# reazon-research/ReazonSpeech

Measured on AMD Instinct MI355X. Metric: RTFx (audio-sec/wall-sec), FastConformer-RNNT 619M batch=256, higher is better.
Workload: dtype bf16

## Files before the change

### reazonspeech_amd/csrc/k_rnnt.hip

```cpp
#include <cstdio>
#include <cstdlib>

#include "k_rnnt_common.h"

namespace {

__global__ void rnnt_init_kernel(DecodeState st, const int32_t* __restrict__ enc_lens, int B, int blank,
                                 int32_t* __restrict__ n_ids) {
    __shared__ int n_alive_s;
    if (threadIdx.x == 0) n_alive_s = 0;
    __syncthreads();
    for (int b = threadIdx.x; b < B; b += blockDim.x) {
        st.tcur[b] = 0; st.sym[b] = 0; st.token[b] = blank; st.act[b] = b;
        if (st.token2) st.token2[b] = -1;
        n_ids[b] = 0;
        if (enc_lens[b] > 0) st.alive[atomicAdd(&n_alive_s, 1)] = b;
    }
    __syncthreads();
    if (threadIdx.x == 0) { st.counters[0] = B; st.counters[1] = 0; st.counters[2] = n_alive_s; st.counters[3] = 0; }
}

__global__ __launch_bounds__(1024) void rnnt_lstm_kernel(DecodeState st, int layer, int B, int H,
                                                        const float* __restrict__ embed,
                                                        const float* __restrict__ W ,
// ... 335 lines not shown
        for (int ctile = lane; ctile < n_ctiles; ctile += 64) {
            const float ov = st.pmax[row * n_ctiles + ctile];
            const int oi = st.pidx[row * n_ctiles + ctile];
            if (ov > val || (ov == val && oi < idx)) { val = ov; idx = oi; }
        }
#pragma unroll
        for (int off = 32; off > 0; off >>= 1) {
            const float ov = __shfl_xor(val, off, 64);
            const int oi = __shfl_xor(idx, off, 64);
            if (ov > val || (ov == val && oi < idx)) { val = ov; idx = oi; }
        }
        if (idx == blank || idx == st.unk || idx == 0x7fffffff) { t += 1; sy = 0; continue; }
        if (lane == 0) {
            const int n = n_ids[b];
            if (n < u_max) { ids[(size_t)b * u_max + n] = idx; frames[(size_t)b * u_max + n] = t; n_ids[b] = n + 1; }
            else st.counters[1] = 1;
            if (st.token2) st.token2[b] = st.token[b];
            st.token[b] = idx;
        }
        emitted = true;
        sy += 1;
        if (sy >= max_symbols) { t += 1; sy = 0; }
        break;
    }
    if (lane != 0) return;
    st.tcur[b] = t; st.sym[b] = sy;
    if (t < T) {
        const int pos = atomicAdd(&st.counters[2 + ((step + 1) & 1)], 1);
        st.alive[(size_t)((step + 1) & 1) * B + pos] = b;
        if (emitted) { const int pa = atomicAdd(&st.counters[0], 1); st.act[pa] = b; }
    }
}

__global__ __launch_bounds__(1024) void rnnt_lstm4_kernel(DecodeState st, int layer, int B, int H,
                                                         const float* __restrict__ embed,
                                                         const float* __restrict__ W4 ,
                                                         const float* __restrict__ bias ) {
    __shared__ float part[SPLITK_LSTM][32][17];
    __shared__ int rows_s[32];
    const int n_act = st.counters[0];
    const int rt = blockIdx.y, ug = blockIdx.x;
    if (rt * 32 >= n_act) return;
    const int tid = threadIdx.x, lane = tid & 63, wave = tid >> 6;
    if (tid < 32) {
        const int i = rt * 32 + tid;
        rows_s[tid] = st.act[i < n_act ? i : n_act - 1];
    }
    __syncthreads();
    const int li = lane & 15, kk = lane >> 4;
    const int lr = lane >> 2, lc = lane & 3;
    const int perm = 4 * (4 * li + kk);
    const int K = 2 * H, kslice = K / SPLITK_LSTM, nkb = K / 16;
    const float* xsrc[2];
    const float* hsrc[2];
#pragma unroll
    for (int ri = 0; ri < 2; ++ri) {
        const int row = rows_s[ri * 16 + lr];
        xsrc[ri] = layer == 0 ? embed + (size_t)st.token[row] * H : st.h_tmp + ((size_t)(layer - 1) * B + row) * H;
        hsrc[ri] = st.h + ((size_t)layer * B + row) * H;
    }
    const float* wfrag = W4 + ((size_t)ug * nkb) * 256 + lane * 4;
    f32x4_t acc[2] = {(f32x4_t){0.f, 0.f, 0.f, 0.f}, (f32x4_t){0.f, 0.f, 0.f, 0.f}};
    const int kbeg = wave * kslice, nblk = kslice / 16;
    float4 av[2][8], wv[8];
#pragma unroll
    for (int u = 0; u < 8; ++u)
        if (u < nblk) {
            const int k = kbeg + 16 * u + 4 * lc;
#pragma unroll
            for (int ri = 0; ri < 2; ++ri)
                av[ri][u] = (k < H) ? *reinterpret_cast<const float4*>(xsrc[ri] + k) : *reinterpret_cast<const float4*>(hsrc[ri] + (k - H));
            wv[u] = *reinterpret_cast<const float4*>(wfrag + (size_t)((kbeg >> 4) + u) * 256);
        }
#pragma unroll
    for (int u = 0; u < 8; ++u)
        if (u < nblk) {
            const float4 a0 = to_mfma_a_layout(av[0][u], perm), a1 = to_mfma_a_layout(av[1][u], perm);
#define RS_MFMA_E(c)                                                                         \
            acc[0] = __builtin_amdgcn_mfma_f32_16x16x4f32(a0.c, wv[u].c, acc[0], 0, 0, 0);   \
            acc[1] = __builtin_amdgcn_mfma_f32_16x16x4f32(a1.c, wv[u].c, acc[1], 0, 0, 0);
            RS_MFMA_E(x) RS_MFMA_E(y) RS_MFMA_E(z) RS_MFMA_E(w)
#undef RS_MFMA_E
        }
#pragma unroll
    for (int ri = 0; ri < 2; ++ri)
#pragma unroll
        for (int r = 0; r < 4; ++r) part[wave][ri * 16 + 4 * kk + r][li] = acc[ri][r];
    __syncthreads();
    if (tid >= 128) return;
    const int i = tid >> 2, u4 = tid & 3;
    if (rt * 32 + i >= n_act) return;
    const int brow = rows_s[i];
    const int unit = ug * 4 + u4;
    float z[4];
#pragma unroll
    for (int gt = 0; gt < 4; ++gt) {
        float sm = part[0][i][gt * 4 + u4];
#pragma unroll
        for (int sl = 1; sl < SPLITK_LSTM; ++sl) sm = sm + part[sl][i][gt * 4 + u4];
        z[gt] = sm + bias[gt * H + unit];
    }
    const float ig = rs_sigmoidf(z[0]), fg = rs_sigmoidf(z[1]), gg = rs_tanhf(z[2]), og = rs_sigmoidf(z[3]);
    const size_t o = ((size_t)layer * B + brow) * H + unit;
    const float cn = fmaf(fg, st.c[o], ig * gg);
    st.c_tmp[o] = cn;
    st.h_tmp[o] = og * rs_tanhf(cn);
}

__global__ __launch_bounds__(512) void rnnt_pred16_kernel(DecodeState st, int B, int L, int H, int N ,
                                                         const float* __restrict__ W, const float* __restrict__ bias) {
    __shared__ float part[SPLITK_TILE][32][17];
    __shared__ int rows_s[32];
    const int rt = blockIdx.y, ct = blockIdx.x;
    const int tid = threadIdx.x, lane = tid & 63, wave = tid >> 6;
    const int n_rows = st.counters[0];
    if (rt * 32 >= n_rows) return;
    if (tid < 32) {
        const int i = rt * 32 + tid;
        rows_s[tid] = st.act[i < n_rows ? i : n_rows - 1];
    }
    __syncthreads();
    const int li = lane & 15, kk = lane >> 4;
    const int lr = lane >> 2, lc = lane & 3;
    const int perm = 4 * (4 * li + kk);
    const int K = H, nkb = K / 16;
    const float* asrc[2];
#pragma unroll
    for (int ri = 0; ri < 2; ++ri) asrc[ri] = st.h_tmp + ((size_t)(L - 1) * B + rows_s[ri * 16 + lr]) * H;
    const float* wfrag = W + ((size_t)ct * nkb) * 256 + lane * 4;
    f32x4_t acc[2] = {(f32x4_t){0.f, 0.f, 0.f, 0.f}, (f32x4_t){0.f, 0.f, 0.f, 0.f}};
    const int kslice = K / SPLITK_TILE, kbeg = wave * kslice, nblk = kslice / 16;
    float4 av[2][8], wv[8];
#pragma unroll
    for (int u = 0; u < 8; ++u)
        if (u < nblk) {
            const int k = kbeg + 16 * u + 4 * lc;
#pragma unroll
            for (int ri = 0; ri < 2; ++ri) av[ri][u] = *reinterpret_cast<const float4*>(asrc[ri] + k);
            wv[u] = *reinterpret_cast<const float4*>(wfrag + (size_t)((kbeg >> 4) + u) * 256);
        }
#pragma unroll
    for (int u = 0; u < 8; ++u)
        if (u < nblk) {
            const float4 a0 = to_mfma_a_layout(av[0][u], perm), a1 = to_mfma_a_layout(av[1][u], perm);
#define RS_MFMA_E(c)                                                                         \
            acc[0] = __builtin_amdgcn_mfma_f32_16x16x4f32(a0.c, wv[u].c, acc[0], 0, 0, 0);   \
            acc[1] = __builtin_amdgcn_mfma_f32_16x16x4f32(a1.c, wv[u].c, acc[1], 0, 0, 0);
            RS_MFMA_E(x) RS_MFMA_E(y) RS_MFMA_E(z) RS_MFMA_E(w)
#undef RS_MFMA_E
        }
#pragma unroll
    for (int ri = 0; ri < 2; ++ri)
#pragma unroll
        for (int r = 0; r < 4; ++r) part[wave][ri * 16 + 4 * kk + r][li] = acc[ri][r];
    __syncthreads();
    const int i = tid >> 4, c = tid & 15;
    const bool row_ok = rt * 32 + i < n_rows;
    const int brow = rows_s[i];
    const int v = ct * 16 + c;
    if (row_ok && v < N) {
        float sm = part[0][i][c];
#pragma unroll
        for (int sl = 1; sl < SPLITK_TILE; ++sl) sm = sm + part[sl][i][c];
        st.g[(size_t)brow * N + v] = sm + bias[v];
    }
    if (row_ok) {
        const int nct = gridDim.x;
        for (int l = 0; l < L; ++l)
            for (int u = ct * 16 + c; u < H; u += nct * 16) {
                const size_t o = ((size_t)l * B + brow) * H + u;
                st.h[o] = st.h_tmp[o];
                st.c[o] = st.c_tmp[o];
            }
    }
}

__global__ __launch_bounds__(256) void rnnt_prep_kernel(DecodeState st, const float* __restrict__ f, int B, int Tp, int J,
                                                        int step) {
    const int lane = threadIdx.x & 63;
    const int slot = blockIdx.x * 4 + (threadIdx.x >> 6);
    if (blockIdx.x == 0 && threadIdx.x == 0) {
        st.counters[0] = 0;
        st.counters[2 + ((step + 1) & 1)] = 0;
    }
    if (slot >= st.counters[2 + (step & 1)]) return;
    const int b = st.alive[(size_t)(step & 1) * B + slot];
    int t = st.tcur[b];
    t = t < Tp ? t : Tp - 1;
    const float* fr = f + ((size_t)b * Tp + t) * J;
    const float* gr = st.g + (size_t)b * J;
    float ss = 0.0f;
    for (int k = 4 * lane; k < J; k += 256) {
        const float4 fv = *reinterpret_cast<const float4*>(fr + k), gv = *reinterpret_cast<const float4*>(gr + k);
        float a0, a1, a2, a3;
        if (st.joint_act) {
            a0 = rs_tanhf(fv.x + gv.x); a1 = rs_tanhf(fv.y + gv.y); a2 = rs_tanhf(fv.z + gv.z); a3 = rs_tanhf(fv.w + gv.w);
        } else {
            a0 = fmaxf(fv.x + gv.x, 0.0f); a1 = fmaxf(fv.y + gv.y, 0.0f); a2 = fmaxf(fv.z + gv.z, 0.0f); a3 = fmaxf(fv.w + gv.w, 0.0f);
        }
        ss = fmaf(a0, a0, fmaf(a1, a1, fmaf(a2, a2, fmaf(a3, a3, ss))));
        *reinterpret_cast<u16x4_t*>(st.a16 + (size_t)slot * J + k) = pack_bf16x4(a0, a1, a2, a3);
    }
    ss = wave_sum(ss);
    if (lane == 0) st.anorm[slot] = sqrtf(ss) * 1.0001f;
}

__global__ __launch_bounds__(256) void rnnt_screen_kernel(DecodeState st, const float* __restrict__ f, int B, int Tp, int J,
                                                          int Vpad, const uint16_t* __restrict__ W16,
                                                          const float* __restrict__ bpad, int step) {
    extern __shared__ __attribute__((aligned(16))) char scr_smem[];
    const int ldrow = J * 2 + 16;
    const int ct = blockIdx.x, rt = blockIdx.y;
    const int tid = threadIdx.x, lane = tid & 63, wave = tid >> 6;
    const int n_alive = st.counters[2 + (step & 1)];
    if (rt * 32 >= n_alive) return;
    const int col0 = (ct * 4 + wave) * 16;
    const bool has_cols = col0 < Vpad;
    const int li = lane & 15, kc = lane >> 4;
    const int nks = J / 32;
    const uint16_t* wrow = W16 + (size_t)((has_cols ? col0 : 0) + li) * J + kc * 8;
    bf16x8_t wf[20];
#pragma unroll
    for (int q = 0; q < 20; ++q)
        if (q < nks) wf[q] = *reinterpret_cast<const bf16x8_t*>(wrow + q * 32);
    const float bv = bpad[(has_cols ? col0 : 0) + li];
    {
        const int per_row = J / 8;
        for (int idx = tid; idx < 32 * per_row; idx += 256) {
            const int r = idx / per_row, c = idx - r * per_row;
            const int i = rt * 32 + r;
            const uint4 v = *reinterpret_cast<const uint4*>(st.a16 + (size_t)(i < n_alive ? i : n_alive - 1) * J + c * 8);
            *reinterpret_cast<uint4*>(scr_smem + r * ldrow + c * 16) = v;
        }
    }
    __syncthreads();
    if (!has_cols) return;
    f32x4_t acc[2] = {(f32x4_t){0.f, 0.f, 0.f, 0.f}, (f32x4_t){0.f, 0.f, 0.f, 0.f}};
#pragma unroll
    for (int q = 0; q < 20; ++q)
        if (q < nks) {
#pragma unroll
            for (int ri = 0; ri < 2; ++ri) {
                const bf16x8_t af = *reinterpret_cast<const bf16x8_t*>(scr_smem + (ri * 16 + li) * ldrow + (q * 32 + kc * 8) * 2);
                acc[ri] = __builtin_amdgcn_mfma_f32_16x16x32_bf16(af, wf[q], acc[ri], 0, 0, 0);
            }
        }
#pragma unroll
    for (int ri = 0; ri < 2; ++ri)
#pragma unroll
        for (int r = 0; r < 4; ++r) {
            const int slot = rt * 32 + ri * 16 + 4 * kc + r;
            if (slot < n_alive) st.zapprox[(size_t)slot * Vpad + col0 + li] = acc[ri][r] + bv;
        }
}

constexpr int VER_CAP = 1024;

__device__ __forceinline__ void verify_evaluate(const int* cand_s, int n_cand, const float* a_s, const float* __restrict__ Wrm,
                                                const float* __restrict__ bo, int J, int lane, float& best, int& best_idx) {
    const int cgrp = lane >> 3, sl = lane & 7;
    const int kslice = J / SPLITK_TILE, nblk = kslice / 16;
    for (int c0 = 0; c0 < n_cand; c0 += 8) {
        const bool valid = c0 + cgrp < n_cand;
        const int cand = valid ? cand_s[c0 + cgrp] : 0;
        const float* w = Wrm + (size_t)cand * J + sl * kslice;
        const float* as = a_s + sl * kslice;
        float4 wv[8][4];
#pragma unroll
        for (int u = 0; u < 8; ++u)
            if (u < nblk) {
#pragma unroll
                for (int kk = 0; kk < 4; ++kk) wv[u][kk] = *reinterpret_cast<const float4*>(w + 16 * u + 4 * kk);
            }
        float acc = 0.0f;
#pragma unroll
        for (int u = 0; u < 8; ++u)
            if (u < nblk) {
                float4 av[4];
#pragma unroll
                for (int kk = 0; kk < 4; ++kk) av[kk] = *reinterpret_cast<const float4*>(as + 16 * u + 4 * kk);
#define RS_CHAIN_E(cc) _Pragma("unroll") for (int kk = 0; kk < 4; ++kk) acc = fmaf(av[kk].cc, wv[u][kk].cc, acc);
                RS_CHAIN_E(x) RS_CHAIN_E(y) RS_CHAIN_E(z) RS_CHAIN_E(w)
#undef RS_CHAIN_E
            }
        float sum = __shfl(acc, lane & ~7, 64);
#pragma unroll
// ... 150 lines not shown
    int n_cand = 0;
#pragma unroll
    for (int c = 0; c < NCHW; ++c) {
        const bool is = zr[c] >= thr;
        const unsigned long long mask = __ballot(is);
        if (is) cand_s[n_cand + __builtin_popcountll(mask & ((1ull << lane) - 1ull))] = (wave * NCHW + c) * 64 + lane;
        n_cand += __builtin_popcountll(mask);
    }
    __builtin_amdgcn_fence(__ATOMIC_ACQ_REL, "wavefront");
    __builtin_amdgcn_wave_barrier();
    float best = -INFINITY;
    int best_idx = 0x7fffffff;
    verify_evaluate(cand_s, n_cand, a_s, Wrm, bo, J, lane, best, best_idx);
    if (lane == 0) { red[4 + wave] = best; reinterpret_cast<int*>(red)[8 + wave] = best_idx; }
    __syncthreads();
    if (threadIdx.x != 0) return;
#pragma unroll
    for (int w = 0; w < 4; ++w) {
        const float v = red[4 + w];
        const int i = reinterpret_cast<int*>(red)[8 + w];
        if (v > best || (v == best && i < best_idx)) { best = v; best_idx = i; }
    }
    verify_commit(st, b, t, best_idx, enc_lens, B, blank, max_symbols, u_max, step, ids, frames, n_ids);
}

}


namespace {

__global__ __launch_bounds__(256) void k2_decoder_kernel(DecodeState st, int B, int D, const float* __restrict__ embed,
                                                         const float* __restrict__ conv_w ) {
    const int n_rows = st.counters[0];
    if ((int)blockIdx.x >= n_rows) return;
    const int row = st.act[blockIdx.x];
    const int t0 = st.token2[row], t1 = st.token[row];
    for (int c = threadIdx.x; c < D; c += 256) {
        const int g4 = c & ~3;
        float acc = 0.0f;
#pragma unroll
        for (int i = 0; i < 4; ++i) {
            const float e = t0 >= 0 ? embed[(size_t)t0 * D + g4 + i] : 0.0f;
            acc = fmaf(conv_w[(c * 4 + i) * 2 + 0], e, acc);
        }
#pragma unroll
        for (int i = 0; i < 4; ++i) {
            const float e = t1 >= 0 ? embed[(size_t)t1 * D + g4 + i] : 0.0f;
            acc = fmaf(conv_w[(c * 4 + i) * 2 + 1], e, acc);
        }
        st.h_tmp[(size_t)row * D + c] = fmaxf(acc, 0.0f);
    }
}

constexpr int LSTM_LDS = SPLITK_LSTM * 4 * 32 * 16 * 4 + 32 * 4;
constexpr int TILE_LDS = SPLITK_TILE * 32 * 65 * 4 + 32 * 4;

bool narrow_kernels_usable(const rs_ctx* ctx) {
    const int L = ctx->d.pred_layers, H = ctx->d.pred_hidden;
    bool narrow = ctx->decode_narrow;
    for (int l = 0; l < L; ++l) narrow = narrow && ctx->lstm_w4[l] != nullptr;
    return narrow && 2 * H / SPLITK_LSTM / 16 <= 8 && H / SPLITK_TILE / 16 <= 8;
}

void launch_lstm_pred(rs_ctx* ctx, const DecodeState& st, int B, int rows_bound, bool narrow, hipStream_t s) {
    const int L = ctx->d.pred_layers, H = ctx->d.pred_hidden, J = ctx->d.joint_hidden;
    const int rts = (rows_bound + 31) / 32 > 0 ? (rows_bound + 31) / 32 : 1;
    if (ctx->k2_conv_w) {
        hipLaunchKernelGGL(k2_decoder_kernel, dim3(rows_bound > 0 ? rows_bound : 1), dim3(256), 0, s, st, B, H, ctx->embed, ctx->k2_conv_w);
        hipLaunchKernelGGL(rnnt_pred16_kernel, dim3((J + 15) / 16, rts), dim3(512), 0, s, st, B, 1, H, J, ctx->jpred_w, ctx->jpred_b);
        return;
    }
    if (narrow) {
        for (int l = 0; l < L; ++l)
            hipLaunchKernelGGL(rnnt_lstm4_kernel, dim3(H / 4, rts), dim3(1024), 0, s, st, l, B, H, ctx->embed, ctx->lstm_w4[l],
                               ctx->lstm_b[l]);
        hipLaunchKernelGGL(rnnt_pred16_kernel, dim3((J + 15) / 16, rts), dim3(512), 0, s, st, B, L, H, J, ctx->jpred_w,
                           ctx->jpred_b);
        return;
    }
    for (int l = 0; l < L; ++l)
        hipLaunchKernelGGL(rnnt_lstm_kernel, dim3(H / 16, rts), dim3(1024), LSTM_LDS, s, st, l, B, H, ctx->embed,
                           ctx->lstm_w[l], ctx->lstm_b[l]);
    hipLaunchKernelGGL(rnnt_tile_kernel<0>, dim3((J + 63) / 64, rts), dim3(512), TILE_LDS, s, st, (const float*)nullptr, B,
                       0, L, H, H, J, ctx->jpred_w, ctx->jpred_b, 0, 0, 1);
}

int joint_grid_x(int nct, int rts) {
    return rts > 1 && !rs_knob(RS_KNOB_DECODE_NO_XCD) ? (nct + 7) / 8 * 8 : nct;
}

int ensure_decode_lds(rs_ctx* ctx) {
    if (int rc = rs_ensure_dynamic_lds(ctx, (const void*)rnnt_lstm_kernel, LSTM_LDS); rc != RS_OK) return rc;
    if (int rc = rs_ensure_dynamic_lds(ctx, (const void*)rnnt_tile_kernel<0>, TILE_LDS); rc != RS_OK) return rc;
    if (int rc = rs_ensure_dynamic_lds(ctx, (const void*)rnnt_tile_kernel<1>, TILE_LDS); rc != RS_OK) return rc;
    if (int rc = rs_ensure_dynamic_lds(ctx, (const void*)rnnt_tile_kernel<2>, TILE_LDS); rc != RS_OK) return rc;
    if (int rc = rs_ensure_dynamic_lds(ctx, (const void*)rnnt_tile_kernel<3>, TILE_LDS); rc != RS_OK) return rc;
    if (int rc = rs_ensure_dynamic_lds(ctx, (const void*)rnnt_tile_kernel<4>, TILE_LDS); rc != RS_OK) return rc;
    return rs_ensure_dynamic_lds(ctx, (const void*)rnnt_tile_kernel<5>, TILE_LDS);
}

}

int rs_rnnt_launch_lstm_pred(rs_ctx* ctx, const void* st_ptr, int rows, hipStream_t s) {
    if (int rc = ensure_decode_lds(ctx); rc != RS_OK) return rc;
    launch_lstm_pred(ctx, *reinterpret_cast<const DecodeState*>(st_ptr), rows, rows, narrow_kernels_usable(ctx), s);
    return RS_OK;
}

int rs_rnnt_launch_joint_logits(rs_ctx* ctx, const void* st_ptr, const float* joint_enc, int rows, int tp_max, int rows_per_utt,
                                int step, hipStream_t s) {
    if (int rc = ensure_decode_lds(ctx); rc != RS_OK) return rc;
    const rs_dims& d = ctx->d;
    const int nct = (d.n_logits + 63) / 64;
    hipLaunchKernelGGL(rnnt_tile_kernel<2>, dim3(joint_grid_x(nct, (rows + 31) / 32), (rows + 31) / 32), dim3(512), TILE_LDS, s,
                       *reinterpret_cast<const DecodeState*>(st_ptr), joint_enc, rows, tp_max, d.pred_layers, d.pred_hidden,
                       d.joint_hidden, d.n_logits, ctx->jout_w, ctx->jout_b, nct, step, rows_per_utt);
    return RS_OK;
}

int rs_rnnt_launch_joint_logits_indirect(rs_ctx* ctx, const void* st_ptr, const float* joint_enc, int rows, int rows_bound, int tp_max,
                                         int rows_per_utt, int step, hipStream_t s) {
    if (int rc = ensure_decode_lds(ctx); rc != RS_OK) return rc;
    const rs_dims& d = ctx->d;
    const int nct = (d.n_logits + 63) / 64;
    const int rts = (rows_bound + 31) / 32 > 0 ? (rows_bound + 31) / 32 : 1;
    const DecodeState& st = *reinterpret_cast<const DecodeState*>(st_ptr);
    if (st.a_pre)
        hipLaunchKernelGGL(rnnt_tile_kernel<4>, dim3(joint_grid_x(nct, rts), rts), dim3(512), TILE_LDS, s, st, joint_enc, rows, tp_max,
                           d.pred_layers, d.pred_hidden, d.joint_hidden, d.n_logits, ctx->jout_w, ctx->jout_b, nct, step, rows_per_utt);
    else
        hipLaunchKernelGGL(rnnt_tile_kernel<3>, dim3(joint_grid_x(nct, rts), rts), dim3(512), TILE_LDS, s, st, joint_enc, rows, tp_max,
                           d.pred_layers, d.pred_hidden, d.joint_hidden, d.n_logits, ctx->jout_w, ctx->jout_b, nct, step, rows_per_utt);
    return RS_OK;
}

constexpr int LOOKAHEAD_MAX = 8;

static void greedy_layout(const rs_ctx* ctx, int B, rs_arena& a, DecodeState& st) {
    const rs_dims& d = ctx->d;
    const size_t state = (size_t)d.pred_layers * B * d.pred_hidden, J = d.joint_hidden;
    const size_t nct = (d.n_logits + 63) / 64, Vpad = (size_t)(d.n_logits + 15) / 16 * 16;
    st.h = a.take<float>(state); st.c = a.take<float>(state);
    st.h_tmp = a.take<float>(state); st.c_tmp = a.take<float>(state);
    st.g = a.take<float>(B * J);
    st.tcur = a.take<int32_t>(B); st.sym = a.take<int32_t>(B);
    st.token = a.take<int32_t>(B); st.act = a.take<int32_t>(B);
    if (ctx->k2_conv_w) st.token2 = a.take<int32_t>(B);
    st.alive = a.take<int32_t>((size_t)2 * B);
    st.counters = a.take<int32_t>(16);
    st.pmax = a.take<float>(B * LOOKAHEAD_MAX * nct); st.pidx = a.take<int32_t>(B * LOOKAHEAD_MAX * nct);
    st.a16 = a.take<uint16_t>(B * J); st.anorm = a.take<float>(B);
    st.zapprox = a.take<float>(B * Vpad);
}
constexpr size_t GREEDY_SLACK = 1024;

size_t rs_rnnt_workspace_bytes(const rs_ctx* ctx, int B) {
    rs_arena a;
    DecodeState st{};
    greedy_layout(ctx, B, a, st);
    return a.bytes() + GREEDY_SLACK;
}

int rs_rnnt_greedy_impl(rs_ctx* ctx, const float* joint_enc, const int32_t* enc_lens, int B, int tp_max, int u_max,
                        int32_t* ids, int32_t* frames, int32_t* n_ids, void* workspace, size_t workspace_bytes,
                        hipStream_t s) {
    const rs_dims& d = ctx->d;
    const int L = d.pred_layers, H = d.pred_hidden, J = d.joint_hidden, V = d.n_logits;
    if (B <= 0) return RS_OK;
    if (H % 128 || J % 128) return rs_fail(ctx, RS_EINVAL, "rnnt: pred_hidden/joint_hidden must be multiples of 128");
    if (L < 1 || L > 4) return rs_fail(ctx, RS_EINVAL, "rnnt: 1..4 LSTM layers supported");
    rs_arena arena(workspace);
    DecodeState st{};
    greedy_layout(ctx, B, arena, st);
    if (workspace_bytes < arena.bytes() + GREEDY_SLACK) return rs_fail(ctx, RS_EWORKSPACE, "rnnt: workspace too small");
    st.joint_act = d.joint_act;
    if (ctx->k2_conv_w) st.unk = ctx->k2 ? rs_k2_unk_id(ctx) : -1;
    const size_t state_bytes = (size_t)L * B * H * 4;
    const int nct = (V + 63) / 64, Vpad = (V + 15) / 16 * 16;
    const bool screen = ctx->decode_screen && ctx->jout_w16 && ctx->jout_wrm && ctx->jout_bpad && ctx->jout_wmax &&
                        J / SPLITK_TILE / 16 <= 8 && J / 32 <= 20;

    if (int rc = ensure_decode_lds(ctx); rc != RS_OK) return rc;
    const bool narrow = narrow_kernels_usable(ctx);
    auto lstm_and_pred = [&](int rows_bound) { launch_lstm_pred(ctx, st, B, rows_bound, narrow, s); };

    rs_prof_begin(ctx, RS_PROF_DECODE, s, 0.0, 0.0);
    RS_HIP(ctx, hipMemsetAsync(st.h, 0, 2 * rs_align(state_bytes), s));
    RS_HIP(ctx, hipMemsetAsync(st.g, 0, (size_t)B * J * 4, s));
    hipLaunchKernelGGL(rnnt_init_kernel, dim3(1), dim3(256), 0, s, st, enc_lens, B, d.blank_id, n_ids);
    lstm_and_pred(B);
    RS_CHECK_LAUNCH(ctx, "rnnt init");

    const int max_steps = tp_max + (u_max < tp_max * d.max_symbols ? u_max : tp_max * d.max_symbols) + 1;
    const int CHUNK = 16;
    const bool lookahead = !rs_knob(RS_KNOB_DECODE_NO_LOOKAHEAD);
    const bool verify_wide = rs_knob(RS_KNOB_VERIFY_WIDE) != 0;
    int32_t host_counters[4] = {0, 0, 0, 0};
    int steps = 0, alive_bound = B;
    bool finished = false;
    while (!finished && steps < max_steps) {
        for (int c = 0; c < CHUNK; ++c, ++steps) {
            const int rows = alive_bound < B ? alive_bound : B;
            if (screen) {
                const int rts = (rows + 31) / 32 > 0 ? (rows + 31) / 32 : 1;
                hipLaunchKernelGGL(rnnt_prep_kernel, dim3((rows + 3) / 4 > 0 ? (rows + 3) / 4 : 1), dim3(256), 0, s, st, joint_enc, B,
                                   tp_max, J, steps);
                hipLaunchKernelGGL(rnnt_screen_kernel, dim3((Vpad + 63) / 64, rts), dim3(256), 32 * (J * 2 + 16), s, st, joint_enc, B,
                                   tp_max, J, Vpad, ctx->jout_w16, ctx->jout_bpad, steps);
                const dim3 vg((rows + 3) / 4 > 0 ? (rows + 3) / 4 : 1), vgw(rows > 0 ? rows : 1);
#define RS_VERIFY_ARGS st, joint_enc, enc_lens, B, tp_max, J, V, Vpad, ctx->jout_wrm, ctx->jout_b, ctx->jout_wmax, d.blank_id, d.max_symbols, u_max, steps, ids, frames, n_ids
                if (V > 64 * 48 && V <= 4 * 64 * 48)
                    hipLaunchKernelGGL(rnnt_verify_wide_kernel<48>, vgw, dim3(256), J * 4 + 4 * 48 * 64 * 4 + 64, s, RS_VERIFY_ARGS);
                else if (V > 64 * 48)
                    hipLaunchKernelGGL(rnnt_verify_kernel<0>, vg, dim3(256), 4 * J * 4 + 4 * VER_CAP * 4, s, RS_VERIFY_ARGS);
                else if (verify_wide)
                    hipLaunchKernelGGL(rnnt_verify_wide_kernel<12>, vgw, dim3(256), J * 4 + 4 * 12 * 64 * 4 + 64, s, RS_VERIFY_ARGS);
                else if (V <= 64 * 8)
                    hipLaunchKernelGGL(rnnt_verify_kernel<8>, vg, dim3(256), 4 * J * 4 + 4 * 8 * 64 * 4, s, RS_VERIFY_ARGS);
                else
                    hipLaunchKernelGGL(rnnt_verify_kernel<48>, vg, dim3(256), 4 * J * 4 + 4 * 48 * 64 * 4, s, RS_VERIFY_ARGS);
#undef RS_VERIFY_ARGS
            } else {
                int la = 1;
                if (lookahead) while (la < LOOKAHEAD_MAX && 2 * la * (rows > 0 ? rows : 1) <= 256) la *= 2;
                if (la > 1) {
                    const int rts = (rows * la + 31) / 32 > 0 ? (rows * la + 31) / 32 : 1;
                    hipLaunchKernelGGL(rnnt_tile_kernel<5>, dim3(joint_grid_x(nct, rts), rts), dim3(512), TILE_LDS, s, st, joint_enc, B, tp_max, L, H,
                                       J, V, ctx->jout_w, ctx->jout_b, nct, steps, la);
                    hipLaunchKernelGGL(rnnt_finalize_la_kernel, dim3((rows + 3) / 4 > 0 ? (rows + 3) / 4 : 1), dim3(256), 0, s, st, enc_lens, B, nct,
                                       d.blank_id, d.max_symbols, u_max, steps, la, ids, frames, n_ids);
                } else {
                    const int rts = (rows + 31) / 32 > 0 ? (rows + 31) / 32 : 1;
                    hipLaunchKernelGGL(rnnt_tile_kernel<1>, dim3(joint_grid_x(nct, rts), rts), dim3(512), TILE_LDS, s, st, joint_enc, B, tp_max, L, H,
                                       J, V, ctx->jout_w, ctx->jout_b, nct, steps, 1);
                    hipLaunchKernelGGL(rnnt_finalize_kernel, dim3((rows + 3) / 4 > 0 ? (rows + 3) / 4 : 1), dim3(256), 0, s, st, enc_lens, B, nct,
                                       d.blank_id, d.max_symbols, u_max, steps, ids, frames, n_ids);
                }
// ... 16 lines not shown
```

### reazonspeech_amd/csrc/rs_knobs.h

```cpp
#pragma once
#include <stdlib.h>
#include <string.h>

#include <atomic>
#include <mutex>

#include "../../include/rs_asr.h"

#define RS_KNOBS(X)                                                                                                                   \
    X(GEMM_TILE, "RS_GEMM_TILE", INT, 0, "forced GEMM tile height (256 / 192 / 128 / 64); 0 = by shape")                              \
    X(GEMM_GROUP_M, "RS_GEMM_GROUP_M", INT, 0, "row panels per XCD tile group; 0 = by shape")                                         \
    X(GEMM_PAIRS, "RS_GEMM_PAIRS", INT, 2, "2 = two tiles per workgroup, LDS ring carried over; 1 = ring restarted; 0 = one tile")    \
    X(GEMM_BREG, "RS_GEMM_BREG", INT, 0, "1 = 256- / 192-row launches keep the weight operand out of LDS (global -> VGPR)")           \
    X(ATTN_PERSIST, "RS_ATTN_PERSIST", INT, 0, "1 = full attention on resident workgroups that walk the items (n >= 2: on n)")        \
    X(ATTN_STREAM, "RS_ATTN_STREAM", INT, 0, "1 = the streaming attention form (+ 16 x mask: phases left out, for timing)")           \
    X(ATTN64, "RS_ATTN64", INT, 4, "head_dim 64: key blocks per chunk; 0 = the one-workgroup-per-CU geometry")                        \
    X(ATTN64_NW, "RS_ATTN64_NW", INT, 4, "head_dim 64: waves per workgroup (the second number of $RS_ATTN64)")                        \
    X(ATTN_F32_OLD, "RS_ATTN_F32_OLD", PRESENT, 0, "float32 attention: the first form (one wave per key sum)")                        \
    X(ATTN_F32_KEYS, "RS_ATTN_F32_KEYS", PRESENT, 0, "float32 attention: the second form (keys over lanes, no MFMA)")                 \
    X(GLU_GENERIC, "RS_GLU_GENERIC", INT, 0, "GLU + depthwise conv: 1 = the any-kernel-size path, 2 = the f32-tile kernel on the gated layout") \
    X(SUB_IM2COL, "RS_SUB_IM2COL", PRESENT, 0, "ESPnet subsampling: gather the 3 x 3 patches into a matrix first (sizes the workspace too)") \
    X(FUSE_GLU, "RS_FUSE_GLU", INT, 1, "context default: 0 = GLU in the depthwise kernel, not the pw1 GEMM epilogue")                 \
    X(DEFER_OUT_NORM, "RS_DEFER_OUT_NORM", INT, 1, "context default: 0 = every output norm stores its f32 rows")                      \
    X(DECODE_SCREEN, "RS_DECODE_SCREEN", INT, 1, "context default: 0 = exact evaluation of every joint column")                       \
    X(DECODE_NARROW, "RS_DECODE_NARROW", INT, 1, "context default: 0 = the wide-tile LSTM / projection kernels")                      \
    X(DECODE_NO_XCD, "RS_DECODE_NO_XCD", PRESENT, 0, "greedy decode: joint grids not padded to a multiple of 8 column tiles")         \
    X(DECODE_NO_LOOKAHEAD, "RS_DECODE_NO_LOOKAHEAD", PRESENT, 0, "greedy decode: one frame per utterance and step at every batch size") \
    X(VERIFY_WIDE, "RS_VERIFY_WIDE", INT, 0, "screened joint: 1 = a workgroup per row for V <= 3072 too")                             \
    X(DECODE_TRACE, "RS_DECODE_TRACE", PRESENT, 0, "greedy decode: print the step count of every call to stderr")                     \
    X(BEAM_SPEC, "RS_BEAM_SPEC", INT, 3, "beam search: evaluations asked for per iteration (1 .. 8; sizes the workspace too)")         \
    X(BEAM_TRACE, "RS_BEAM_TRACE", PRESENT, 0, "beam search: phase timing of the step kernel")                                        \
    X(BEAM_RECORD_LDS, "RS_BEAM_RECORD_LDS", PRESENT, 0, "beam search: the any-vocabulary record kernel on a small vocabulary")       \
    X(AVSR_POSCONV_OLD, "RS_AVSR_POSCONV_OLD", PRESENT, 0, "AV-HuBERT positional convolution: the VALU form")                         \
    X(K2_CONV1_OLD, "RS_K2_CONV1_OLD", PRESENT, 0, "Zipformer conv1: the VALU form (the one other channel counts run)")               \
    X(K2_ATTW_SWEEPS, "RS_K2_ATTW_SWEEPS", INT, 1, "Zipformer attention weights: 3 = the three-sweep kernel")                         \
    X(K2_CONV2_FUSED, "RS_K2_CONV2_FUSED", INT, 1, "default of option k2_conv2_fused: 0 = patch matrix + GEMM launch")                \
    X(K2_CNX_FUSED, "RS_K2_CNX_FUSED", INT, 1, "default of option k2_cnx_fused: 0 = the ConvNeXt pointwise pair as two GEMM launches")

enum rs_knob_id {
#define RS_KNOB_ENUM(id, env, kind, def, what) RS_KNOB_##id,
    RS_KNOBS(RS_KNOB_ENUM)
#undef RS_KNOB_ENUM
    RS_KNOB_COUNT
};
enum rs_knob_kind { RS_KNOB_PRESENT, RS_KNOB_INT };
struct rs_knob_row { const char* env; rs_knob_kind kind; int def; };
static const rs_knob_row rs_knob_rows[RS_KNOB_COUNT] = {
#define RS_KNOB_ROW(id, env, kind, def, what) {env, RS_KNOB_##kind, def},
    RS_KNOBS(RS_KNOB_ROW)
#undef RS_KNOB_ROW
};

struct rs_knob_table {
    std::atomic<int> value[RS_KNOB_COUNT];
    std::atomic<bool> given[RS_KNOB_COUNT];
    std::once_flag once;
};
inline rs_knob_table rs_knob_state;

inline void rs_knobs_read_env() {
// ... 38 lines not shown
```

Baseline: 46360.

## Loop decode kernels over row tiles to reuse register-held weights across tiles

```diff
diff --git a/reazonspeech_amd/csrc/k_rnnt.hip b/reazonspeech_amd/csrc/k_rnnt.hip
--- a/reazonspeech_amd/csrc/k_rnnt.hip
+++ b/reazonspeech_amd/csrc/k_rnnt.hip
@@ -391,6 +391,7 @@
     }
 }
 
+constexpr int LSTM4_NB = 5;
 __global__ __launch_bounds__(1024) void rnnt_lstm4_kernel(DecodeState st, int layer, int B, int H,
                                                          const float* __restrict__ embed,
                                                          const float* __restrict__ W4 ,
@@ -398,139 +399,163 @@
     __shared__ float part[SPLITK_LSTM][32][17];
     __shared__ int rows_s[32];
     const int n_act = st.counters[0];
-    const int rt = blockIdx.y, ug = blockIdx.x;
-    if (rt * 32 >= n_act) return;
+    const int ug = blockIdx.x;
+    if ((int)blockIdx.y * 32 >= n_act) return;
     const int tid = threadIdx.x, lane = tid & 63, wave = tid >> 6;
-    if (tid < 32) {
-        const int i = rt * 32 + tid;
-        rows_s[tid] = st.act[i < n_act ? i : n_act - 1];
-    }
-    __syncthreads();
     const int li = lane & 15, kk = lane >> 4;
     const int lr = lane >> 2, lc = lane & 3;
     const int perm = 4 * (4 * li + kk);
     const int K = 2 * H, kslice = K / SPLITK_LSTM, nkb = K / 16;
-    const float* xsrc[2];
-    const float* hsrc[2];
-#pragma unroll
-    for (int ri = 0; ri < 2; ++ri) {
-        const int row = rows_s[ri * 16 + lr];
-        xsrc[ri] = layer == 0 ? embed + (size_t)st.token[row] * H : st.h_tmp + ((size_t)(layer - 1) * B + row) * H;
-        hsrc[ri] = st.h + ((size_t)layer * B + row) * H;
-    }
-    const float* wfrag = W4 + ((size_t)ug * nkb) * 256 + lane * 4;
-    f32x4_t acc[2] = {(f32x4_t){0.f, 0.f, 0.f, 0.f}, (f32x4_t){0.f, 0.f, 0.f, 0.f}};
     const int kbeg = wave * kslice, nblk = kslice / 16;
-    float4 av[2][8], wv[8];
-#pragma unroll
-    for (int u = 0; u < 8; ++u)
-        if (u < nblk) {
-            const int k = kbeg + 16 * u + 4 * lc;
-#pragma unroll
-            for (int ri = 0; ri < 2; ++ri)
-                av[ri][u] = (k < H) ? *reinterpret_cast<const float4*>(xsrc[ri] + k) : *reinterpret_cast<const float4*>(hsrc[ri] + (k - H));
-            wv[u] = *reinterpret_cast<const float4*>(wfrag + (size_t)((kbeg >> 4) + u) * 256);
-        }
-#pragma unroll
-    for (int u = 0; u < 8; ++u)
-        if (u < nblk) {
-            const float4 a0 = to_mfma_a_layout(av[0][u], perm), a1 = to_mfma_a_layout(av[1][u], perm);
-#define RS_MFMA_E(c)                                                                         \
-            acc[0] = __builtin_amdgcn_mfma_f32_16x16x4f32(a0.c, wv[u].c, acc[0], 0, 0, 0);   \
-            acc[1] = __builtin_amdgcn_mfma_f32_16x16x4f32(a1.c, wv[u].c, acc[1], 0, 0, 0);
-            RS_MFMA_E(x) RS_MFMA_E(y) RS_MFMA_E(z) RS_MFMA_E(w)
+    int my_row = 0;
+    if (tid < 32) {
+        const int i = blockIdx.y * 32 + tid;
+        my_row = st.act[i < n_act ? i : n_act - 1];
+    }
+    constexpr int NB = LSTM4_NB;
+    const float* wfrag = W4 + ((size_t)ug * nkb + (kbeg >> 4)) * 256 + lane * 4;
+    float4 wv[NB];
+#pragma unroll
+    for (int u = 0; u < NB; ++u)
+        if (u < nblk) wv[u] = *reinterpret_cast<const float4*>(wfrag + u * 256);
+#pragma clang loop unroll(disable)
+    for (int rt = blockIdx.y; rt * 32 < n_act; rt += gridDim.y) {
+        const bool more = (rt + (int)gridDim.y) * 32 < n_act;
+        if (tid < 32) rows_s[tid] = my_row;
+        __syncthreads();
+        const float* asrc[2];
+#pragma unroll
+        for (int ri = 0; ri < 2; ++ri) {
+            const int row = rows_s[ri * 16 + lr];
+            if (kbeg < H)
+                asrc[ri] = (layer == 0 ? embed + (size_t)st.token[row] * H : st.h_tmp + ((size_t)(layer - 1) * B + row) * H) + kbeg + 4 * lc;
+            else
+                asrc[ri] = st.h + ((size_t)layer * B + row) * H + (kbeg - H) + 4 * lc;
+        }
+        f32x4_t acc[2] = {(f32x4_t){0.f, 0.f, 0.f, 0.f}, (f32x4_t){0.f, 0.f, 0.f, 0.f}};
+        float4 av[2][NB];
+#pragma unroll
+        for (int u = 0; u < NB; ++u)
+            if (u < nblk) {
+#pragma unroll
+                for (int ri = 0; ri < 2; ++ri) av[ri][u] = *reinterpret_cast<const float4*>(asrc[ri] + 16 * u);
+            }
+        if (more && tid < 32) {
+            const int i = (rt + gridDim.y) * 32 + tid;
+            my_row = st.act[i < n_act ? i : n_act - 1];
+        }
+#pragma unroll
+        for (int u = 0; u < NB; ++u)
+            if (u < nblk) {
+                const float4 a0 = to_mfma_a_layout(av[0][u], perm), a1 = to_mfma_a_layout(av[1][u], perm);
+#define RS_MFMA_E(c)                                                                             \
+                acc[0] = __builtin_amdgcn_mfma_f32_16x16x4f32(a0.c, wv[u].c, acc[0], 0, 0, 0);   \
+                acc[1] = __builtin_amdgcn_mfma_f32_16x16x4f32(a1.c, wv[u].c, acc[1], 0, 0, 0);
+                RS_MFMA_E(x) RS_MFMA_E(y) RS_MFMA_E(z) RS_MFMA_E(w)
 #undef RS_MFMA_E
-        }
-#pragma unroll
-    for (int ri = 0; ri < 2; ++ri)
-#pragma unroll
-        for (int r = 0; r < 4; ++r) part[wave][ri * 16 + 4 * kk + r][li] = acc[ri][r];
-    __syncthreads();
-    if (tid >= 128) return;
-    const int i = tid >> 2, u4 = tid & 3;
-    if (rt * 32 + i >= n_act) return;
-    const int brow = rows_s[i];
-    const int unit = ug * 4 + u4;
-    float z[4];
-#pragma unroll
-    for (int gt = 0; gt < 4; ++gt) {
-        float sm = part[0][i][gt * 4 + u4];
-#pragma unroll
-        for (int sl = 1; sl < SPLITK_LSTM; ++sl) sm = sm + part[sl][i][gt * 4 + u4];
-        z[gt] = sm + bias[gt * H + unit];
-    }
-    const float ig = rs_sigmoidf(z[0]), fg = rs_sigmoidf(z[1]), gg = rs_tanhf(z[2]), og = rs_sigmoidf(z[3]);
-    const size_t o = ((size_t)layer * B + brow) * H + unit;
-    const float cn = fmaf(fg, st.c[o], ig * gg);
-    st.c_tmp[o] = cn;
-    st.h_tmp[o] = og * rs_tanhf(cn);
+            }
+#pragma unroll
+        for (int ri = 0; ri < 2; ++ri)
+#pragma unroll
+            for (int r = 0; r < 4; ++r) part[wave][ri * 16 + 4 * kk + r][li] = acc[ri][r];
+        __syncthreads();
+        const int i = tid >> 2, u4 = tid & 3;
+        if (tid < 128 && rt * 32 + i < n_act) {
+            const int brow = rows_s[i];
+            const int unit = ug * 4 + u4;
+            float z[4];
+#pragma unroll
+            for (int gt = 0; gt < 4; ++gt) {
+                float sm = part[0][i][gt * 4 + u4];
+#pragma unroll
+                for (int sl = 1; sl < SPLITK_LSTM; ++sl) sm = sm + part[sl][i][gt * 4 + u4];
+                z[gt] = sm + bias[gt * H + unit];
+            }
+            const float ig = rs_sigmoidf(z[0]), fg = rs_sigmoidf(z[1]), gg = rs_tanhf(z[2]), og = rs_sigmoidf(z[3]);
+            const size_t o = ((size_t)layer * B + brow) * H + unit;
+            const float cn = fmaf(fg, st.c[o], ig * gg);
+            st.c_tmp[o] = cn;
+            st.h_tmp[o] = og * rs_tanhf(cn);
+        }
+        if (more) __syncthreads();
+    }
 }
 
 __global__ __launch_bounds__(512) void rnnt_pred16_kernel(DecodeState st, int B, int L, int H, int N ,
                                                          const float* __restrict__ W, const float* __restrict__ bias) {
     __shared__ float part[SPLITK_TILE][32][17];
     __shared__ int rows_s[32];
-    const int rt = blockIdx.y, ct = blockIdx.x;
+    const int ct = blockIdx.x;
     const int tid = threadIdx.x, lane = tid & 63, wave = tid >> 6;
     const int n_rows = st.counters[0];
-    if (rt * 32 >= n_rows) return;
-    if (tid < 32) {
-        const int i = rt * 32 + tid;
-        rows_s[tid] = st.act[i < n_rows ? i : n_rows - 1];
-    }
-    __syncthreads();
+    if ((int)blockIdx.y * 32 >= n_rows) return;
     const int li = lane & 15, kk = lane >> 4;
     const int lr = lane >> 2, lc = lane & 3;
     const int perm = 4 * (4 * li + kk);
     const int K = H, nkb = K / 16;
-    const float* asrc[2];
-#pragma unroll
-    for (int ri = 0; ri < 2; ++ri) asrc[ri] = st.h_tmp + ((size_t)(L - 1) * B + rows_s[ri * 16 + lr]) * H;
-    const float* wfrag = W + ((size_t)ct * nkb) * 256 + lane * 4;
-    f32x4_t acc[2] = {(f32x4_t){0.f, 0.f, 0.f, 0.f}, (f32x4_t){0.f, 0.f, 0.f, 0.f}};
     const int kslice = K / SPLITK_TILE, kbeg = wave * kslice, nblk = kslice / 16;
-    float4 av[2][8], wv[8];
+    if (tid < 32) {
+        const int i = blockIdx.y * 32 + tid;
+        rows_s[tid] = st.act[i < n_rows ? i : n_rows - 1];
+    }
+    const float* wfrag = W + ((size_t)ct * nkb + (kbeg >> 4)) * 256 + lane * 4;
+    float4 wv[8];
 #pragma unroll
     for (int u = 0; u < 8; ++u)
-        if (u < nblk) {
-            const int k = kbeg + 16 * u + 4 * lc;
-#pragma unroll
-            for (int ri = 0; ri < 2; ++ri) av[ri][u] = *reinterpret_cast<const float4*>(asrc[ri] + k);
-            wv[u] = *reinterpret_cast<const float4*>(wfrag + (size_t)((kbeg >> 4) + u) * 256);
-        }
-#pragma unroll
-    for (int u = 0; u < 8; ++u)
-        if (u < nblk) {
-            const float4 a0 = to_mfma_a_layout(av[0][u], perm), a1 = to_mfma_a_layout(av[1][u], perm);
-#define RS_MFMA_E(c)                                                                         \
-            acc[0] = __builtin_amdgcn_mfma_f32_16x16x4f32(a0.c, wv[u].c, acc[0], 0, 0, 0);   \
-            acc[1] = __builtin_amdgcn_mfma_f32_16x16x4f32(a1.c, wv[u].c, acc[1], 0, 0, 0);
-            RS_MFMA_E(x) RS_MFMA_E(y) RS_MFMA_E(z) RS_MFMA_E(w)
+        if (u < nblk) wv[u] = *reinterpret_cast<const float4*>(wfrag + u * 256);
+    for (int rt = blockIdx.y; rt * 32 < n_rows; rt += gridDim.y) {
+        const bool more = (rt + (int)gridDim.y) * 32 < n_rows;
+        if (tid < 32 && rt != (int)blockIdx.y) {
+            const int i = rt * 32 + tid;
+            rows_s[tid] = st.act[i < n_rows ? i : n_rows - 1];
+        }
+        __syncthreads();
+        const float* asrc[2];
+#pragma unroll
+        for (int ri = 0; ri < 2; ++ri) asrc[ri] = st.h_tmp + ((size_t)(L - 1) * B + rows_s[ri * 16 + lr]) * H + kbeg + 4 * lc;
+        f32x4_t acc[2] = {(f32x4_t){0.f, 0.f, 0.f, 0.f}, (f32x4_t){0.f, 0.f, 0.f, 0.f}};
+        float4 av[2][8];
+#pragma unroll
+        for (int u = 0; u < 8; ++u)
+            if (u < nblk) {
+#pragma unroll
+                for (int ri = 0; ri < 2; ++ri) av[ri][u] = *reinterpret_cast<const float4*>(asrc[ri] + 16 * u);
+            }
+#pragma unroll
+        for (int u = 0; u < 8; ++u)
+            if (u < nblk) {
+                const float4 a0 = to_mfma_a_layout(av[0][u], perm), a1 = to_mfma_a_layout(av[1][u], perm);
+#define RS_MFMA_E(c)                                                                             \
+                acc[0] = __builtin_amdgcn_mfma_f32_16x16x4f32(a0.c, wv[u].c, acc[0], 0, 0, 0);   \
+                acc[1] = __builtin_amdgcn_mfma_f32_16x16x4f32(a1.c, wv[u].c, acc[1], 0, 0, 0);
+                RS_MFMA_E(x) RS_MFMA_E(y) RS_MFMA_E(z) RS_MFMA_E(w)
 #undef RS_MFMA_E
-        }
-#pragma unroll
-    for (int ri = 0; ri < 2; ++ri)
-#pragma unroll
-        for (int r = 0; r < 4; ++r) part[wave][ri * 16 + 4 * kk + r][li] = acc[ri][r];
-    __syncthreads();
-    const int i = tid >> 4, c = tid & 15;
-    const bool row_ok = rt * 32 + i < n_rows;
-    const int brow = rows_s[i];
-    const int v = ct * 16 + c;
-    if (row_ok && v < N) {
-        float sm = part[0][i][c];
-#pragma unroll
-        for (int sl = 1; sl < SPLITK_TILE; ++sl) sm = sm + part[sl][i][c];
-        st.g[(size_t)brow * N + v] = sm + bias[v];
-    }
-    if (row_ok) {
-        const int nct = gridDim.x;
-        for (int l = 0; l < L; ++l)
-            for (int u = ct * 16 + c; u < H; u += nct * 16) {
-                const size_t o = ((size_t)l * B + brow) * H + u;
-                st.h[o] = st.h_tmp[o];
-                st.c[o] = st.c_tmp[o];
-            }
+            }
+#pragma unroll
+        for (int ri = 0; ri < 2; ++ri)
+#pragma unroll
+            for (int r = 0; r < 4; ++r) part[wave][ri * 16 + 4 * kk + r][li] = acc[ri][r];
+        __syncthreads();
+        const int i = tid >> 4, c = tid & 15;
+        const bool row_ok = rt * 32 + i < n_rows;
+        const int brow = rows_s[i];
+        const int v = ct * 16 + c;
+        if (row_ok && v < N) {
+            float sm = part[0][i][c];
+#pragma unroll
+            for (int sl = 1; sl < SPLITK_TILE; ++sl) sm = sm + part[sl][i][c];
+            st.g[(size_t)brow * N + v] = sm + bias[v];
+        }
+        if (row_ok) {
+            const int nct = gridDim.x;
+            for (int l = 0; l < L; ++l)
+                for (int u = ct * 16 + c; u < H; u += nct * 16) {
+                    const size_t o = ((size_t)l * B + brow) * H + u;
+                    st.h[o] = st.h_tmp[o];
+                    st.c[o] = st.c_tmp[o];
+                }
+        }
+        if (more) __syncthreads();
     }
 }
 
@@ -569,10 +594,10 @@
                                                           const float* __restrict__ bpad, int step) {
     extern __shared__ __attribute__((aligned(16))) char scr_smem[];
     const int ldrow = J * 2 + 16;
-    const int ct = blockIdx.x, rt = blockIdx.y;
+    const int ct = blockIdx.x;
     const int tid = threadIdx.x, lane = tid & 63, wave = tid >> 6;
     const int n_alive = st.counters[2 + (step & 1)];
-    if (rt * 32 >= n_alive) return;
+    if ((int)blockIdx.y * 32 >= n_alive) return;
     const int col0 = (ct * 4 + wave) * 16;
     const bool has_cols = col0 < Vpad;
     const int li = lane & 15, kc = lane >> 4;
@@ -583,34 +608,38 @@
     for (int q = 0; q < 20; ++q)
         if (q < nks) wf[q] = *reinterpret_cast<const bf16x8_t*>(wrow + q * 32);
     const float bv = bpad[(has_cols ? col0 : 0) + li];
-    {
-        const int per_row = J / 8;
-        for (int idx = tid; idx < 32 * per_row; idx += 256) {
-            const int r = idx / per_row, c = idx - r * per_row;
-            const int i = rt * 32 + r;
-            const uint4 v = *reinterpret_cast<const uint4*>(st.a16 + (size_t)(i < n_alive ? i : n_alive - 1) * J + c * 8);
-            *reinterpret_cast<uint4*>(scr_smem + r * ldrow + c * 16) = v;
-        }
-    }
-    __syncthreads();
-    if (!has_cols) return;
-    f32x4_t acc[2] = {(f32x4_t){0.f, 0.f, 0.f, 0.f}, (f32x4_t){0.f, 0.f, 0.f, 0.f}};
-#pragma unroll
-    for (int q = 0; q < 20; ++q)
-        if (q < nks) {
-#pragma unroll
-            for (int ri = 0; ri < 2; ++ri) {
-                const bf16x8_t af = *reinterpret_cast<const bf16x8_t*>(scr_smem + (ri * 16 + li) * ldrow + (q * 32 + kc * 8) * 2);
-                acc[ri] = __builtin_amdgcn_mfma_f32_16x16x32_bf16(af, wf[q], acc[ri], 0, 0, 0);
-            }
-        }
-#pragma unroll
-    for (int ri = 0; ri < 2; ++ri)
-#pragma unroll
-        for (int r = 0; r < 4; ++r) {
-            const int slot = rt * 32 + ri * 16 + 4 * kc + r;
-            if (slot < n_alive) st.zapprox[(size_t)slot * Vpad + col0 + li] = acc[ri][r] + bv;
-        }
+    for (int rt = blockIdx.y; rt * 32 < n_alive; rt += gridDim.y) {
+        {
+            const int per_row = J / 8;
+            for (int idx = tid; idx < 32 * per_row; idx += 256) {
+                const int r = idx / per_row, c = idx - r * per_row;
+                const int i = rt * 32 + r;
+                const uint4 v = *reinterpret_cast<const uint4*>(st.a16 + (size_t)(i < n_alive ? i : n_alive - 1) * J + c * 8);
+                *reinterpret_cast<uint4*>(scr_smem + r * ldrow + c * 16) = v;
+            }
+        }
+        __syncthreads();
+        if (has_cols) {
+            f32x4_t acc[2] = {(f32x4_t){0.f, 0.f, 0.f, 0.f}, (f32x4_t){0.f, 0.f, 0.f, 0.f}};
+#pragma unroll
+            for (int q = 0; q < 20; ++q)
+                if (q < nks) {
+#pragma unroll
+                    for (int ri = 0; ri < 2; ++ri) {
+                        const bf16x8_t af = *reinterpret_cast<const bf16x8_t*>(scr_smem + (ri * 16 + li) * ldrow + (q * 32 + kc * 8) * 2);
+                        acc[ri] = __builtin_amdgcn_mfma_f32_16x16x32_bf16(af, wf[q], acc[ri], 0, 0, 0);
+                    }
+                }
+#pragma unroll
+            for (int ri = 0; ri < 2; ++ri)
+#pragma unroll
+                for (int r = 0; r < 4; ++r) {
+                    const int slot = rt * 32 + ri * 16 + 4 * kc + r;
+                    if (slot < n_alive) st.zapprox[(size_t)slot * Vpad + col0 + li] = acc[ri][r] + bv;
+                }
+        }
+        if ((rt + (int)gridDim.y) * 32 < n_alive) __syncthreads();
+    }
 }
 
 constexpr int VER_CAP = 1024;
@@ -827,23 +856,24 @@
 __global__ __launch_bounds__(256) void k2_decoder_kernel(DecodeState st, int B, int D, const float* __restrict__ embed,
                                                          const float* __restrict__ conv_w ) {
     const int n_rows = st.counters[0];
-    if ((int)blockIdx.x >= n_rows) return;
-    const int row = st.act[blockIdx.x];
-    const int t0 = st.token2[row], t1 = st.token[row];
-    for (int c = threadIdx.x; c < D; c += 256) {
-        const int g4 = c & ~3;
-        float acc = 0.0f;
-#pragma unroll
-        for (int i = 0; i < 4; ++i) {
-            const float e = t0 >= 0 ? embed[(size_t)t0 * D + g4 + i] : 0.0f;
-            acc = fmaf(conv_w[(c * 4 + i) * 2 + 0], e, acc);
-        }
-#pragma unroll
-        for (int i = 0; i < 4; ++i) {
-            const float e = t1 >= 0 ? embed[(size_t)t1 * D + g4 + i] : 0.0f;
-            acc = fmaf(conv_w[(c * 4 + i) * 2 + 1], e, acc);
-        }
-        st.h_tmp[(size_t)row * D + c] = fmaxf(acc, 0.0f);
+    for (int r = blockIdx.x; r < n_rows; r += gridDim.x) {
+        const int row = st.act[r];
+        const int t0 = st.token2[row], t1 = st.token[row];
+        for (int c = threadIdx.x; c < D; c += 256) {
+            const int g4 = c & ~3;
+            float acc = 0.0f;
+#pragma unroll
+            for (int i = 0; i < 4; ++i) {
+                const float e = t0 >= 0 ? embed[(size_t)t0 * D + g4 + i] : 0.0f;
+                acc = fmaf(conv_w[(c * 4 + i) * 2 + 0], e, acc);
+            }
+#pragma unroll
+            for (int i = 0; i < 4; ++i) {
+                const float e = t1 >= 0 ? embed[(size_t)t1 * D + g4 + i] : 0.0f;
+                acc = fmaf(conv_w[(c * 4 + i) * 2 + 1], e, acc);
+            }
+            st.h_tmp[(size_t)row * D + c] = fmaxf(acc, 0.0f);
+        }
     }
 }
 
@@ -854,22 +884,26 @@
     const int L = ctx->d.pred_layers, H = ctx->d.pred_hidden;
     bool narrow = ctx->decode_narrow;
     for (int l = 0; l < L; ++l) narrow = narrow && ctx->lstm_w4[l] != nullptr;
-    return narrow && 2 * H / SPLITK_LSTM / 16 <= 8 && H / SPLITK_TILE / 16 <= 8;
-}
-
-void launch_lstm_pred(rs_ctx* ctx, const DecodeState& st, int B, int rows_bound, bool narrow, hipStream_t s) {
+    return narrow && 2 * H / SPLITK_LSTM / 16 <= LSTM4_NB && H / SPLITK_TILE / 16 <= 8;
+}
+
+int row_tiles(int rows) { return (rows + 31) / 32 > 0 ? (rows + 31) / 32 : 1; }
+
+void launch_lstm_pred(rs_ctx* ctx, const DecodeState& st, int B, int rows_bound, int lanes, bool narrow, hipStream_t s) {
     const int L = ctx->d.pred_layers, H = ctx->d.pred_hidden, J = ctx->d.joint_hidden;
-    const int rts = (rows_bound + 31) / 32 > 0 ? (rows_bound + 31) / 32 : 1;
+    const int rts = row_tiles(rows_bound);
+    const int ly = lanes < 1 ? 1 : lanes < rts ? lanes : rts;
     if (ctx->k2_conv_w) {
-        hipLaunchKernelGGL(k2_decoder_kernel, dim3(rows_bound > 0 ? rows_bound : 1), dim3(256), 0, s, st, B, H, ctx->embed, ctx->k2_conv_w);
-        hipLaunchKernelGGL(rnnt_pred16_kernel, dim3((J + 15) / 16, rts), dim3(512), 0, s, st, B, 1, H, J, ctx->jpred_w, ctx->jpred_b);
+        const int nwg = rows_bound < ly * 32 ? rows_bound : ly * 32;
+        hipLaunchKernelGGL(k2_decoder_kernel, dim3(nwg > 0 ? nwg : 1), dim3(256), 0, s, st, B, H, ctx->embed, ctx->k2_conv_w);
+        hipLaunchKernelGGL(rnnt_pred16_kernel, dim3((J + 15) / 16, ly), dim3(512), 0, s, st, B, 1, H, J, ctx->jpred_w, ctx->jpred_b);
         return;
     }
     if (narrow) {
         for (int l = 0; l < L; ++l)
-            hipLaunchKernelGGL(rnnt_lstm4_kernel, dim3(H / 4, rts), dim3(1024), 0, s, st, l, B, H, ctx->embed, ctx->lstm_w4[l],
+            hipLaunchKernelGGL(rnnt_lstm4_kernel, dim3(H / 4, ly), dim3(1024), 0, s, st, l, B, H, ctx->embed, ctx->lstm_w4[l],
                                ctx->lstm_b[l]);
-        hipLaunchKernelGGL(rnnt_pred16_kernel, dim3((J + 15) / 16, rts), dim3(512), 0, s, st, B, L, H, J, ctx->jpred_w,
+        hipLaunchKernelGGL(rnnt_pred16_kernel, dim3((J + 15) / 16, ly), dim3(512), 0, s, st, B, L, H, J, ctx->jpred_w,
                            ctx->jpred_b);
         return;
     }
@@ -898,7 +932,7 @@
 
 int rs_rnnt_launch_lstm_pred(rs_ctx* ctx, const void* st_ptr, int rows, hipStream_t s) {
     if (int rc = ensure_decode_lds(ctx); rc != RS_OK) return rc;
-    launch_lstm_pred(ctx, *reinterpret_cast<const DecodeState*>(st_ptr), rows, rows, narrow_kernels_usable(ctx), s);
+    launch_lstm_pred(ctx, *reinterpret_cast<const DecodeState*>(st_ptr), rows, rows, row_tiles(rows), narrow_kernels_usable(ctx), s);
     return RS_OK;
 }
 
@@ -930,6 +964,8 @@
 }
 
 constexpr int LOOKAHEAD_MAX = 8;
+constexpr int DECODE_ACT_ROW_LANES = 99;
+constexpr int DECODE_ALIVE_ROW_LANES = 99;
 
 static void greedy_layout(const rs_ctx* ctx, int B, rs_arena& a, DecodeState& st) {
     const rs_dims& d = ctx->d;
@@ -977,7 +1013,13 @@
 
     if (int rc = ensure_decode_lds(ctx); rc != RS_OK) return rc;
     const bool narrow = narrow_kernels_usable(ctx);
-    auto lstm_and_pred = [&](int rows_bound) { launch_lstm_pred(ctx, st, B, rows_bound, narrow, s); };
+    const int lanes_knob = rs_knob(RS_KNOB_DECODE_ROW_LANES);
+    auto row_lanes = [&](int rts, bool act_rows) {
+        if (lanes_knob > 0) return lanes_knob < rts ? lanes_knob : rts;
+        if (lanes_knob < 0) return act_rows && -lanes_knob < rts ? -lanes_knob : rts;
+        return rts <= 2 ? rts : act_rows ? DECODE_ACT_ROW_LANES : DECODE_ALIVE_ROW_LANES;
+    };
+    auto lstm_and_pred = [&](int rows_bound) { launch_lstm_pred(ctx, st, B, rows_bound, row_lanes(row_tiles(rows_bound), true), narrow, s); };
 
     rs_prof_begin(ctx, RS_PROF_DECODE, s, 0.0, 0.0);
     RS_HIP(ctx, hipMemsetAsync(st.h, 0, 2 * rs_align(state_bytes), s));
@@ -997,7 +1039,7 @@
         for (int c = 0; c < CHUNK; ++c, ++steps) {
             const int rows = alive_bound < B ? alive_bound : B;
             if (screen) {
-                const int rts = (rows + 31) / 32 > 0 ? (rows + 31) / 32 : 1;
+                const int rts = row_lanes(row_tiles(rows), false);
                 hipLaunchKernelGGL(rnnt_prep_kernel, dim3((rows + 3) / 4 > 0 ? (rows + 3) / 4 : 1), dim3(256), 0, s, st, joint_enc, B,
                                    tp_max, J, steps);
                 hipLaunchKernelGGL(rnnt_screen_kernel, dim3((Vpad + 63) / 64, rts), dim3(256), 32 * (J * 2 + 16), s, st, joint_enc, B,
diff --git a/reazonspeech_amd/csrc/rs_knobs.h b/reazonspeech_amd/csrc/rs_knobs.h
--- a/reazonspeech_amd/csrc/rs_knobs.h
+++ b/reazonspeech_amd/csrc/rs_knobs.h
@@ -26,6 +26,7 @@
     X(DECODE_NARROW, "RS_DECODE_NARROW", INT, 1, "context default: 0 = the wide-tile LSTM / projection kernels")                      \
     X(DECODE_NO_XCD, "RS_DECODE_NO_XCD", PRESENT, 0, "greedy decode: joint grids not padded to a multiple of 8 column tiles")         \
     X(DECODE_NO_LOOKAHEAD, "RS_DECODE_NO_LOOKAHEAD", PRESENT, 0, "greedy decode: one frame per utterance and step at every batch size") \
+    X(DECODE_ROW_LANES, "RS_DECODE_ROW_LANES", INT, 0, "greedy decode: workgroups per column tile that walk its row tiles; 0 = by rule, n = at most n, -n = LSTM / projection only") \
     X(VERIFY_WIDE, "RS_VERIFY_WIDE", INT, 0, "screened joint: 1 = a workgroup per row for V <= 3072 too")                             \
     X(DECODE_TRACE, "RS_DECODE_TRACE", PRESENT, 0, "greedy decode: print the step count of every call to stderr")                     \
     X(BEAM_SPEC, "RS_BEAM_SPEC", INT, 3, "beam search: evaluations asked for per iteration (1 .. 8; sizes the workspace too)")         \
```

Result: no change. 46050 (-0.7%).
